# aidanmrli/rwm-pt-pytorch

Hardware: AMD Instinct MI355X
Metric: chain-MH-steps/sec (higher is better)
Workload: dtype f32; 1 GPU; BASELINE configs[2]: PT-RWM HIP, RoughCarpet dim=30 modes[-15,0,15], Normal proposal 2.38^2/dim, 32 geometric temps 1->0.01, swap_every=10, 65536 ladders per GPU; dim=30, temps=32, ladders_per_gpu=65536, mh_steps_per_launch=2000, swap_every=10, swap_mode=exchange, swap_order=sequential, rng=Philox4x32-10 in-kernel, world_size=1

## Files before the change

### include/ptrwm.h

```cpp
#ifndef PTRWM_H
#define PTRWM_H

#include <stdint.h>

#ifdef __cplusplus
extern "C" {
#endif

#define PTRWM_ABI_VERSION 3
#define PTRWM_SPLIT_NO_SWEEP 1
#define PTRWM_MAX_DIM 104
#define PTRWM_MAX_TEMPS 256

enum {
  PTRWM_OK = 0,
  PTRWM_E_NULL = -1,
  PTRWM_E_DIM = -2,
  PTRWM_E_TEMPS = -3,
  PTRWM_E_KIND = -4,
  PTRWM_E_ARG = -5,
  PTRWM_E_STRUCT = -6,
  PTRWM_E_LAUNCH = -7,
  PTRWM_E_NOVARIANT = -8
};
// ... 140 lines not shown
  uint32_t struct_size;
  int32_t temps;
  int32_t every;
  double *sum;
  double *sum_sq;
  double *sum_logp;
  int64_t *count;
} ptrwm_chain_moments_args;

int32_t ptrwm_run_with_chain_moments(const ptrwm_target_desc *target, const ptrwm_proposal_desc *proposal,
                                     const ptrwm_run_args *args, const ptrwm_chain_moments_args *chain_moments, void *stream);

int32_t ptrwm_split_chain_moments(const ptrwm_run_args *args, int32_t dim, const ptrwm_chain_moments_args *chain_moments,
                                  void *stream);

int32_t ptrwm_swap_sweep(const ptrwm_run_args *args, int32_t dim, int64_t event_index, int32_t rng_stream,
                         void *stream);

int32_t ptrwm_split_propose(const ptrwm_proposal_desc *proposal, const ptrwm_run_args *args, int32_t dim,
                            float *proposals, float *accept_u, void *stream);
int32_t ptrwm_split_accept(const ptrwm_run_args *args, int32_t dim, float *proposals, const float *accept_u,
                           const float *logp_proposed, void *stream);
int32_t ptrwm_split_advance(const ptrwm_run_args *args, void *stream);

int32_t ptrwm_logdensity(const ptrwm_target_desc *target, const float *x, float *out, int64_t n,
                         void *stream);

int32_t ptrwm_propose(const ptrwm_proposal_desc *proposal, int32_t dim, int32_t n_temps, int64_t n,
                      const float *ext_raw, uint64_t seed, float *out, void *stream);

int32_t ptrwm_philox_raw(uint64_t seed, uint32_t c0, uint32_t c1, uint32_t c2, uint32_t c3,
                         int64_t n, uint32_t *out, void *stream);

int32_t ptrwm_has_variant(int32_t target_kind, int32_t proposal_kind, int32_t dim);

int32_t ptrwm_abi_version(void);
const char *ptrwm_strerror(int32_t code);

#ifdef __cplusplus
}
#endif
#endif
```

### rwm-pt-pytorch_amd/csrc/capi.hip

```cpp
#include <algorithm>
#include <cmath>

#include "../../include/ptrwm.h"
#include "variants.h"

namespace ptrwm {

struct VariantPair {
  const TargetVariants *narrow, *wide;
  RunLaunchFn run(int proposal, int dpi) const {
    const RunLaunchFn f = narrow->run[proposal][dpi];
    return f != nullptr ? f : wide->run[proposal][dpi];
  }
  LogpLaunchFn logp(int dpi) const {
    const LogpLaunchFn f = narrow->logp[dpi];
    return f != nullptr ? f : wide->logp[dpi];
  }
};

#include "form_table.inc"

static void form_lerp(const float *a, const float *b, float t, float *out, int n) {
  for (int i = 0; i < n; ++i) out[i] = a[i] + (b[i] - a[i]) * t;
}
// ... 216 lines not shown
}

static int specialised_form(const ptrwm_target_desc *t, int perm[3]) {
  if (t->kind == PTRWM_TARGET_ROUGH_CARPET) return rough_carpet_fold(t->p, perm) ? 2 : (rough_carpet_two_term(t->p) ? 1 : 0);
  if (t->kind == PTRWM_TARGET_THREE_MIXTURE) return t->ip[0] == 1 ? 1 : 0;
  return 0;
}

static TParams make_tparams(const ptrwm_target_desc *t) {
  TParams tp;
  for (int i = 0; i < 12; ++i) tp.p[i] = t->p[i];
  for (int i = 0; i < 4; ++i) tp.ip[i] = t->ip[i];
  tp.vec0 = t->vec0;
  tp.vec1 = t->vec1;
  tp.mask[0] = tp.mask[1] = 0;
  if (t->kind == PTRWM_TARGET_ROUGH_CARPET) {
    tp.p[7] = -(float)t->dim * 0.91893853320467274178f;
  }
  if (t->kind == PTRWM_TARGET_HYBRID_ROSENBROCK) {
    const int blk = t->ip[0] - 1;
    for (int i = 1; i < t->dim; ++i)
      if ((i - 1) % blk == 0) tp.mask[i >> 6] |= (1ull << (i & 63));
  }
  return tp;
}

__global__ void split_advance_kernel(long long *device_step, long long n) { *device_step += n; }

__global__ void philox_raw_kernel(uint32_t *__restrict__ out, long long n, uint32_t c0, uint32_t c1, uint32_t c2,
                                  uint32_t c3, uint32_t k0, uint32_t k1) {
  const long long i = (long long)blockIdx.x * blockDim.x + threadIdx.x;
  if (i >= n) return;
  const u32x4 r = philox4x32_10(c0 + (uint32_t)i, c1, c2, c3, k0, k1);
  out[4 * i + 0] = r.x;
  out[4 * i + 1] = r.y;
  out[4 * i + 2] = r.z;
  out[4 * i + 3] = r.w;
}

struct SweepArgs {
  float *state, *logp;
  const float *beta, *ext_swap_u;
  long long *swap_accept, *last_swap_ordinal;
  const float *prev;
  double *sq_jump;
  long long chain_offset, event_index;
  unsigned long long step;
  int n_temps, dim, swap_mode, swap_order, rng_stream, chunk;
  unsigned k0, k1;
  const long long *device_step;
  long long burn_in, swap_every, event_offset;
};
constexpr int kSweepLdsBytes = 32768;

template <class state_t>
__global__ void __launch_bounds__(256) swap_sweep_kernel(SweepArgs a) {
  if (a.device_step != nullptr) {
    const long long s0 = *a.device_step + (long long)a.step, sc = s0 + 1;
    if (!(sc > a.burn_in && sc % a.swap_every == 0)) return;
    a.step = (unsigned long long)s0;
    a.event_index = sc / a.swap_every - a.burn_in / a.swap_every - 1 + a.event_offset;
  }
  extern __shared__ __attribute__((aligned(16))) unsigned char s_sweep[];
  __shared__ float s_l[256], s_u[256];
  __shared__ int s_src[256];
  const int T = a.n_temps, D = a.dim, tid = threadIdx.x, nthr = blockDim.x;
// ... 831 lines not shown
  const int dpi = width_index_for_dim(dim);
  if (dpi < 0) return PTRWM_E_DIM;
  PParams pp;
  pp.dim_scale = proposal->dim_scale;
  pp.inv_dim = proposal->inv_dim;
  const int n_raw = ptrwm_ext_raw_per_step(proposal->kind, dim);
  const unsigned k0 = (unsigned)(seed & 0xffffffffull), k1 = (unsigned)(seed >> 32);
  hipError_t err;
  switch (proposal->kind) {
    case PTRWM_PROPOSAL_NORMAL:
      err = launch_propose<NormalProposal>(dpi, out, n, dim, n_temps, proposal->temp_scale, pp, ext_raw, n_raw, k0, k1, (hipStream_t)stream);
      break;
    case PTRWM_PROPOSAL_LAPLACE:
      err = launch_propose<LaplaceProposal>(dpi, out, n, dim, n_temps, proposal->temp_scale, pp, ext_raw, n_raw, k0, k1, (hipStream_t)stream);
      break;
    default:
      err = launch_propose<UniformRadiusProposal>(dpi, out, n, dim, n_temps, proposal->temp_scale, pp, ext_raw, n_raw, k0, k1, (hipStream_t)stream);
      break;
  }
  return err == hipSuccess ? PTRWM_OK : PTRWM_E_LAUNCH;
}

int32_t ptrwm_philox_raw(uint64_t seed, uint32_t c0, uint32_t c1, uint32_t c2, uint32_t c3, int64_t n, uint32_t *out,
                         void *stream) {
  if (n < 0) return PTRWM_E_ARG;
  if (n == 0) return PTRWM_OK;
  if (out == nullptr) return PTRWM_E_NULL;
  const unsigned grid = (unsigned)((n + 255) / 256);
  hipLaunchKernelGGL(philox_raw_kernel, dim3(grid), dim3(256), 0, (hipStream_t)stream, out, (long long)n, c0, c1, c2,
                     c3, (unsigned)(seed & 0xffffffffull), (unsigned)(seed >> 32));
  return hipGetLastError() == hipSuccess ? PTRWM_OK : PTRWM_E_LAUNCH;
}

}
```

### rwm-pt-pytorch_amd/csrc/kernel.h

```cpp
#pragma once
#include "philox.h"
#include "proposals.h"
#include "targets.h"

namespace ptrwm {

#ifndef PTRWM_BLOCK_THREADS
#define PTRWM_BLOCK_THREADS 256
#endif
constexpr int kBlockThreads = PTRWM_BLOCK_THREADS;
constexpr int kWavesPerBlock = kBlockThreads / 64;
struct StepLdsWords {
  static constexpr int kSwapWords = 3;
  static constexpr int kParkedInts = 3;
  static constexpr int kExtraPerThread = kSwapWords + kParkedInts + 2;
  static constexpr int kStreamSlabs = 2;
  static constexpr int kStreamStatPerThread = 5;
  static constexpr unsigned kVoteBytes = 16u;
  static constexpr int floats_per_thread(int dp, bool stream) { return (stream ? kStreamSlabs * (dp + kStreamStatPerThread) : dp) + kExtraPerThread; }
  static constexpr unsigned bytes(int threads, int dp, bool stream, bool wide) { return (unsigned)(threads * floats_per_thread(dp, stream)) * 4u + (wide ? kVoteBytes : 0u); }
};
template <int DP, bool STREAM = false>
struct StepLds : StepLdsWords {
  static constexpr int kWaveFloats = 64 * floats_per_thread(DP, STREAM);
// ... 279 lines not shown
      else sum_logp[row0 + i] = reg[2 * rd + i];
    }
}

template <bool EXACT>
__device__ __forceinline__ int fresh_dim(int d0) {
  if constexpr (!EXACT) PTRWM_VALUE_BARRIER("+s"(d0));
  return d0;
}

typedef const __attribute__((address_space(4))) KArgs *kargs_ptr;
__device__ __forceinline__ kargs_ptr late_args() {
  uintptr_t p = (uintptr_t)__builtin_amdgcn_kernarg_segment_ptr();
  PTRWM_VALUE_BARRIER("+s"(p));
  return (kargs_ptr)p;
}

#ifndef PTRWM_J2_FENCE_MASK
#define PTRWM_J2_FENCE_MASK 7
#endif
#ifndef PTRWM_WAVES_SMALL
#define PTRWM_WAVES_SMALL 4
#endif
#ifndef PTRWM_WAVES_40
#define PTRWM_WAVES_40 3
#endif
#ifndef PTRWM_WAVES_MID
#define PTRWM_WAVES_MID 2
#endif
constexpr int min_waves_per_simd(int dp) {
  return dp <= 30 ? PTRWM_WAVES_SMALL : (dp <= 44 ? PTRWM_WAVES_40 : (dp <= 64 ? PTRWM_WAVES_MID : 1));
}
constexpr bool step_loop_at_register_cap(int dp, bool stream) { return !stream && min_waves_per_simd(dp) >= 4 && dp > 24; }

constexpr int stream_waves_per_simd(int dp) {
  return dp <= 10 ? 4 : (dp <= 20 ? 2 : (dp <= 30 ? 2 : 1));
}

constexpr int stream_register_waves(int dp) { return stream_waves_per_simd(dp) < 2 ? 2 : stream_waves_per_simd(dp); }

template <class Target, class Proposal, int DP, bool EXACT, bool FULL, bool STREAM = false>
__global__ void __launch_bounds__(kBlockThreads, STREAM ? stream_register_waves(DP) : min_waves_per_simd(DP)) ptrwm_step_kernel(const KArgs a) {
  static_assert(!(STREAM && FULL), "the streaming form is a production kernel: no fixture / trace arguments");
  const int T = a.n_temps;
  const int D0 = EXACT ? DP : a.dim;
  const int cpw = a.chains_per_wave;
  const bool wide = !STREAM && T > 64;
  const int wave = wave_in_block();
  const int tid = wide ? (int)threadIdx.x : (int)(threadIdx.x & 63);
  long long group = STREAM ? (long long)blockIdx.x * kWavesPerBlock + wave
                           : (wide ? (long long)blockIdx.x : (long long)blockIdx.x * kWavesPerBlock + (threadIdx.x >> 6));
  [[maybe_unused]] const long long n_groups = STREAM ? a.n_chains / cpw : 0;
  [[maybe_unused]] const long long group_stride = STREAM ? (long long)gridDim.x * kWavesPerBlock : 0;
  if (STREAM ? (group >= n_groups) : (group * cpw >= a.n_chains)) return;
  extern __shared__ __attribute__((aligned(16))) float s_dyn[];
  typedef float pf_vec4 __attribute__((ext_vector_type(4)));
  typedef StepLds<DP, STREAM> L;
  constexpr int NV = STREAM ? L::kSlabVectorsPerLane : 1;
  constexpr int kWaveFloats = L::kWaveFloats;
  [[maybe_unused]] int cur = 0;
  typedef const __attribute__((address_space(1))) void *dma_src;
  typedef __attribute__((address_space(3))) void *dma_dst;
  [[maybe_unused]] auto prefetch = [&](long long g, int slab) {
    const int tid = thread_index_now(wave) & 63;
    const kargs_ptr ap = late_args();
    const int n_vec = (cpw * T * D0) >> 2;
// ... 98 lines not shown
    }
    if constexpr (STREAM) asm volatile("s_waitcnt vmcnt(0)" ::: "memory");
    sync_group();
    const float *row = s_stage + row_head + (live ? tid : 0) * D0;
#pragma unroll
    for (int d = 0; d < DP; ++d) x[d] = (d < D0) ? row[d] : 0.0f;
  }
  float lp;
  [[maybe_unused]] double sq_old = 0.0;
  [[maybe_unused]] long long acc_old = 0;
  if constexpr (STREAM) {
    {
      const float *zone = s_dyn + wave * kWaveFloats + L::zone(cur);
      lp = (zone + L::kZoneLogp)[tid];
      if (a.sq_jump != nullptr) sq_old = reinterpret_cast<const double *>(zone + L::kZoneSqJump)[tid < cpw * T ? tid : 0];
      if (a.n_accept != nullptr) acc_old = reinterpret_cast<const long long *>(zone + L::kZoneAccept)[tid < cpw * T ? tid : 0];
    }
    if (have_pending) flush_pending();
    if (group + group_stride < n_groups) prefetch(group + group_stride, cur ^ 1);
  } else {
    lp = a.logp[rep];
  }
  const float beta_t = STREAM ? beta_t_s : a.beta[t];
  const float tscale = STREAM ? tscale_s : a.temp_scale[t];
  bool jump_trusted = false;
  if constexpr (Proposal::kKnowsJump) {
    float xmax = 0.0f;
#pragma unroll
    for (int d = 0; d < DP; ++d) xmax = __builtin_fmaxf(xmax, __builtin_fabsf(x[d]));
    jump_trusted = xmax <= kJumpTrust * Proposal::increment_scale(tscale, a.pp);
  }

  const unsigned long long gchain = (unsigned long long)(a.chain_offset + chain);
  RngCtx rc;
  rc.c2 = (uint32_t)gchain;
  rc.k0 = a.k0;
  rc.k1 = a.k1;
  const uint32_t c3_base = (uint32_t)t | ((uint32_t)(gchain >> 32) << 12);

  unsigned n_acc = 0;
  {
    const int gt = wide ? ((T + 63) & ~63) : 64;
    int *const park = reinterpret_cast<int *>(STREAM ? s_dyn + wave * kWaveFloats + L::parked(gt) : s_stage + L::parked(gt)) + tid;
    park[0] = (int)c3_base;
    park[L::kSwapCount * gt] = 0;
    park[L::kLastEvent * gt] = -1;
    reinterpret_cast<double *>(park - tid + L::kSqJump * gt)[tid] = 0.0;
  }

  const bool ext = FULL && a.full.ext_prop != nullptr;
  const bool trace_on =
      FULL && live && a.full.trace != nullptr && (chain < a.full.trace_chains) && (t < a.full.trace_temps);
  int to_swap = a.steps_to_swap;
  int to_trace = FULL ? a.full.steps_to_trace : 0;
  [[maybe_unused]] int to_mom = FULL ? a.full.steps_to_mom : 0;
  int trace_rows = 0;
  int swap_in_call = 0;
  const int ev_par0 = (int)(a.first_swap_event & 1);
  unsigned long long s = (unsigned long long)a.step0;

  constexpr int W = canon_width(DP);
  auto commit_plain = [&](bool acc, float jump, int jump_kind, int D) __attribute__((always_inline)) -> float {
    float j2;
    if (jump_kind != kJumpNone) {
      float from_states = 0.0f;
      if (!jump_trusted) {
        PTRWM_COLD_PATH();
        float j2p[4] = {0.0f, 0.0f, 0.0f, 0.0f};
        PTRWM_DIM_LOOP(d, DP, D, {
          const float dl = sub_rn(y[d], x[d]);
          j2p[d / W] = fmaf(dl, dl, j2p[d / W]);
        })
        from_states = tree4_add(j2p);
      }
      PTRWM_DIM_LOOP(d, DP, D, {
        x[d] = acc ? y[d] : x[d];
        if ((d & PTRWM_J2_FENCE_MASK) == PTRWM_J2_FENCE_MASK) sched_fence_soft();
      })
      j2 = acc ? (jump_trusted ? jump : from_states) : 0.0f;
    } else {
      float j2p[4] = {0.0f, 0.0f, 0.0f, 0.0f};
      PTRWM_DIM_LOOP(d, DP, D, {
        const float dl = sub_rn(y[d], x[d]);
        j2p[d / W] = fmaf(dl, dl, j2p[d / W]);
        x[d] = acc ? y[d] : x[d];
        if ((d & PTRWM_J2_FENCE_MASK) == PTRWM_J2_FENCE_MASK) sched_fence_soft();
      })
      j2 = tree4_add(j2p);
      if (!acc) j2 = 0.0f;
    }
    return j2;
  };
// ... 29 lines not shown
        if (mom_now && count_on && live && t < a.full.mom_temps) {
          const int mt = a.full.mom_temps, pc = a.full.mom_chain;
          const int m_rows = moments_rows(pc != 0, cpw, mt), m_row = pc != 0 ? cw * mt + t : t;
          double *const reg = L::moments_region(s_dyn, wide, wide ? ((T + 63) & ~63) : 64, wave, (int)moments_region_doubles(m_rows, D));
          double *const rs = reg + m_row * D;
          double *const rq = reg + (m_rows + m_row) * D;
          PTRWM_DIM_LOOP(d, DP, D, {
            const double v = (double)x[d];
            moments_add(rs + d, v);
            moments_add(rq + d, v * v);
          })
          moments_add(reg + 2 * m_rows * D + m_row, (double)lp);
        }
      }
    }
  };

  int i = 0;
  while (i < a.n_steps) {
    const int left = a.n_steps - i;
    const bool to_multiple = to_swap <= left;
    int run = to_multiple ? to_swap : left;
    to_swap = to_multiple ? a.swap_every : to_swap - left;
    bool count_on, acc;
    float lp_mh;
    float jump;
    int jump_kind;
    int D;
    for (;; ++i, ++s) {
      count_on = i >= a.burn_left;
      rc.c0hi = (uint32_t)(s >> 32) << 16;
      rc.c1 = (uint32_t)s;
      rc.c3 = c3_base | (kStreamMH << 8);
      if constexpr (step_loop_at_register_cap(DP, STREAM)) asm volatile("" : "+v"(rc.c2));

      long long srep = 0;
      const float *ext_raw = nullptr;
      float ext_u = 0.0f;
      if constexpr (FULL) {
        srep = ((long long)i * a.n_chains + chain) * T + t;
        if (ext) {
          ext_raw = a.full.ext_prop + srep * a.full.n_raw_ext;
          ext_u = a.full.ext_u[srep];
        }
      }

      jump = 0.0f;
      const float u_acc = Proposal::propose(y, x, fresh_dim<EXACT>(D0), tscale, a.pp, rc, ext_raw, ext_u, jump, jump_kind);
      const float lp_new = Target::template logp<false>(y, fresh_dim<EXACT>(D0), a.tp);
      D = fresh_dim<EXACT>(D0);

      acc = mh_accept(beta_t, lp_new, lp, u_acc);
      lp_mh = acc ? lp_new : lp;
      if constexpr (FULL) {
        if (a.full.accept_flags != nullptr && live) a.full.accept_flags[srep] = acc ? 1 : 0;
      }

      if (--run == 0) break;
      const float j2 = commit_plain(acc, jump, jump_kind, D);
      lp = lp_mh;
      finish_step(count_on, acc, j2, D);
    }
    const bool swap_due = to_multiple && count_on && (T > 1);

    float j2;
    if (!swap_due) {
      j2 = commit_plain(acc, jump, jump_kind, D);
// ... 273 lines not shown
```

### rwm-pt-pytorch_amd/csrc/philox.h

```cpp
#pragma once
#include <hip/hip_runtime.h>
#include <stdint.h>

namespace ptrwm {

struct u32x4 {
  uint32_t x, y, z, w;
};

constexpr uint32_t kPhiloxM0 = 0xD2511F53u;
constexpr uint32_t kPhiloxM1 = 0xCD9E8D57u;
constexpr uint32_t kPhiloxW0 = 0x9E3779B9u;
constexpr uint32_t kPhiloxW1 = 0xBB67AE85u;

constexpr uint32_t kStreamMH = 0u;
constexpr uint32_t kStreamSwap = 1u;

__device__ __forceinline__ void mul_hilo(uint32_t m, uint32_t x, uint32_t &hi, uint32_t &lo) {
  const uint64_t p = (uint64_t)m * x;
  hi = (uint32_t)(p >> 32);
  lo = (uint32_t)p;
}

__device__ __forceinline__ u32x4 philox4x32_10(uint32_t c0, uint32_t c1, uint32_t c2, uint32_t c3,
                                               uint32_t k0, uint32_t k1) {
#pragma unroll
  for (int r = 0; r < 10; ++r) {
    uint32_t hi0, lo0, hi1, lo1;
    mul_hilo(kPhiloxM0, c0, hi0, lo0);
    mul_hilo(kPhiloxM1, c2, hi1, lo1);
    uint32_t n0, n2;
    if (r >= 2) {
      n0 = __builtin_amdgcn_bitop3_b32(hi1, c1, k0, 0x96);
      n2 = __builtin_amdgcn_bitop3_b32(hi0, c3, k1, 0x96);
    } else {
      n0 = hi1 ^ c1 ^ k0;
      n2 = hi0 ^ c3 ^ k1;
    }
    c1 = lo1;
    c3 = lo0;
    c0 = n0;
    c2 = n2;
    k0 += kPhiloxW0;
    k1 += kPhiloxW1;
  }
  return u32x4{c0, c1, c2, c3};
}

#ifdef PTRWM_NO_VALUE_BARRIERS
#define PTRWM_VALUE_BARRIER(...) ((void)0)
#else
#define PTRWM_VALUE_BARRIER(...) asm volatile("" : __VA_ARGS__)
#endif

#define PTRWM_COLD_PATH() asm volatile("; ptrwm-cold-path")

typedef const __attribute__((address_space(4))) float *const_float_ptr;
__device__ __forceinline__ const_float_ptr uniform_vec(const float *p) {
  uintptr_t v = (uintptr_t)p;
  PTRWM_VALUE_BARRIER("+s"(v));
  return (const_float_ptr)v;
}

__device__ __forceinline__ const_float_ptr uniform_vec_again(const_float_ptr p) {
  uintptr_t v = (uintptr_t)p;
  PTRWM_VALUE_BARRIER("+s"(v));
  return (const_float_ptr)v;
}

__device__ __forceinline__ float u01(uint32_t r) { return (float)(r >> 8) * 0x1p-24f; }
__device__ __forceinline__ float u01_open0(uint32_t r) {
  return ((float)(r >> 8) + 1.0f) * 0x1p-24f;
}

constexpr float kLn2 = 0.69314718055994530942f;
// ... 60 lines not shown
```

### rwm-pt-pytorch_amd/csrc/proposals.h

```cpp
#pragma once
#include "philox.h"
#include "../../include/ptrwm.h"

namespace ptrwm {

struct RngCtx {
  uint32_t c0hi, c1, c2, c3, k0, k1;
};

enum { kJumpNone = 0, kJumpPartial = 1, kJumpTotal = 2 };
constexpr float kJumpTrust = 256.0f;

struct PParams {
  const float *__restrict__ dim_scale;
  float inv_dim;
};

__device__ __forceinline__ uint32_t pick(const u32x4 &r, int lane4) {
  return lane4 == 0 ? r.x : (lane4 == 1 ? r.y : (lane4 == 2 ? r.z : r.w));
}

template <int DP>
__device__ __forceinline__ void philox_normals(float (&z)[DP], int D, const RngCtx &rc, int w_a,
                                               float &ua, float &ub) {
  constexpr int NB = (2 * ((DP + 1) / 2)) / 4 + 1;
#pragma unroll
  for (int c = 0; c < NB; ++c) {
    if (4 * c + 4 <= DP && 4 * c + 4 <= D) {
      const u32x4 r = philox4x32_10(rc.c0hi | (uint32_t)c, rc.c1, rc.c2, rc.c3, rc.k0, rc.k1);
#pragma unroll
      for (int h = 0; h < 2; ++h) {
        const int d = (4 * c + 2 * h + 1 < DP) ? 4 * c + 2 * h : 0;
        float z0, z1;
        box_muller(h ? r.z : r.x, h ? r.w : r.y, z0, z1);
        z[d] = z0;
        z[d + 1] = z1;
      }
      sched_fence();
    } else if (4 * c <= w_a + 1) {
      const u32x4 r = philox4x32_10(rc.c0hi | (uint32_t)c, rc.c1, rc.c2, rc.c3, rc.k0, rc.k1);
      if (4 * c < DP && 4 * c < D) {
        float z0, z1;
        box_muller(r.x, r.y, z0, z1);
        z[4 * c < DP ? 4 * c : 0] = z0;
        if (4 * c + 1 < DP && 4 * c + 1 < D) z[4 * c + 1 < DP ? 4 * c + 1 : 0] = z1;
      }
      if (4 * c + 2 < DP && 4 * c + 2 < D) {
        float z0, z1;
        box_muller(r.z, r.w, z0, z1);
        z[4 * c + 2 < DP ? 4 * c + 2 : 0] = z0;
        if (4 * c + 3 < DP && 4 * c + 3 < D) z[4 * c + 3 < DP ? 4 * c + 3 : 0] = z1;
      }
      if (4 * c == w_a) {
        ua = u01(r.x);
        ub = u01(r.y);
      }
      if (4 * c + 2 == w_a) {
        ua = u01(r.z);
        ub = u01(r.w);
      }
      sched_fence();
    }
  }
}

template <int DP>
__device__ __forceinline__ float philox_normal_step(float (&y)[DP], const float (&x)[DP], int D, float tscale,
                                                    const RngCtx &rc, float &jump_total) {
  constexpr int W = canon_width(DP);
  float jump[4] = {0.0f, 0.0f, 0.0f, 0.0f};
  const float c_t = mul_rn(mul_rn(-2.0f * kLn2, tscale), tscale);
  constexpr int NB = (2 * ((DP + 1) / 2)) / 4 + 1;
#ifdef PTRWM_INJECT_ACCEPT_WORD_SLIP
  const int w_a = 2 * ((D + 1) >> 1) - 2;
#else
  const int w_a = 2 * ((D + 1) >> 1);
#endif
  float u_acc = 0.0f;
#pragma unroll
  for (int c = 0; c < NB; ++c) {
    if (4 * c + 4 <= DP && 4 * c + 4 <= D) {
      const u32x4 r = philox4x32_10(rc.c0hi | (uint32_t)c, rc.c1, rc.c2, rc.c3, rc.k0, rc.k1);
#pragma unroll
      for (int h = 0; h < 2; ++h) {
        const int d = (4 * c + 2 * h + 1 < DP) ? 4 * c + 2 * h : 0;
        const uint32_t ra = h ? r.z : r.x, rb = h ? r.w : r.y;
        const float arg = mul_rn(c_t, hw_log2(u01_open0(ra)));
        const float rad = hw_sqrt(arg);
        const float ang = bm_turns(rb);
        y[d] = fmaf(rad, __builtin_amdgcn_sinf(ang), x[d]);
        y[d + 1] = fmaf(rad, __builtin_amdgcn_cosf(ang), x[d + 1]);
        jump[d / W] = add_rn(jump[d / W], arg);
      }
      sched_fence();
    } else if (4 * c <= w_a) {
      const u32x4 r = philox4x32_10(rc.c0hi | (uint32_t)c, rc.c1, rc.c2, rc.c3, rc.k0, rc.k1);
#pragma unroll
      for (int h = 0; h < 2; ++h) {
        const int d = 4 * c + 2 * h;
        const uint32_t ra = h ? r.z : r.x, rb = h ? r.w : r.y;
        if (d < DP && d < D) {
          const float arg = mul_rn(c_t, hw_log2(u01_open0(ra)));
          const float rad = hw_sqrt(arg);
          const float ang = bm_turns(rb);
          const int d0 = d < DP ? d : 0, d1 = d + 1 < DP ? d + 1 : 0;
          const float sn = __builtin_amdgcn_sinf(ang);
          y[d0] = fmaf(rad, sn, x[d0]);
          if (d + 1 < DP && d + 1 < D) {
            y[d1] = fmaf(rad, __builtin_amdgcn_cosf(ang), x[d1]);
            jump[d0 / W] = add_rn(jump[d0 / W], arg);
          } else {
            const float i0 = mul_rn(rad, sn);
            jump[d0 / W] = fmaf(i0, i0, jump[d0 / W]);
          }
        }
        if (d == w_a) u_acc = u01(ra);
      }
      sched_fence();
    }
  }
  jump_total = tree4_add(jump);
  return u_acc;
}

template <int DP>
struct NormalProposal {
  static constexpr int kKind = PTRWM_PROPOSAL_NORMAL;
  static constexpr bool kKnowsJump = true;
  __device__ __forceinline__ static float increment_scale(float tscale, const PParams &) { return tscale; }
  __device__ __forceinline__ static float propose(float (&y)[DP], const float (&x)[DP], int D,
                                                  float tscale, const PParams &, const RngCtx &rc,
                                                  const float *ext_raw, float ext_u, float &jump, int &jump_kind) {
    float u_acc = ext_u;
    if (ext_raw != nullptr) {
      jump_kind = kJumpNone;
#pragma unroll
      for (int d = 0; d < DP; ++d)
        if (d < D) y[d] = add_rn(x[d], mul_rn(ext_raw[d], tscale));
    } else {
      jump_kind = kJumpTotal;
      u_acc = philox_normal_step<DP>(y, x, D, tscale, rc, jump);
    }
    return u_acc;
  }
};

template <int DP>
struct LaplaceProposal {
  static constexpr int kKind = PTRWM_PROPOSAL_LAPLACE;
  static constexpr bool kKnowsJump = false;
  __device__ __forceinline__ static float increment_scale(float tscale, const PParams &) { return tscale; }
  __device__ __forceinline__ static float transform(float u01v, float scale) {
    const float u = u01v - 0.5f;
    const float au = __builtin_fabsf(u);
    const float arg = __builtin_fmaxf(-2.0f * au, -0.999999f);
    const float l1p = hw_log2(1.0f + arg) * kLn2;
    const float t = mul_rn(scale, l1p);
    return __builtin_bit_cast(float, __builtin_amdgcn_bitop3_b32(__builtin_bit_cast(uint32_t, t),
                                                                 __builtin_bit_cast(uint32_t, u), 0x80000000u, 0xd2));
  }
  __device__ __forceinline__ static float propose(float (&y)[DP], const float (&x)[DP], int D,
                                                  float tscale, const PParams &pp, const RngCtx &rc,
                                                  const float *ext_raw, float ext_u, float &, int &jump_kind) {
    float u_acc = ext_u;
    jump_kind = kJumpNone;
    const const_float_ptr dsc = uniform_vec(pp.dim_scale);
    if (ext_raw != nullptr) {
#pragma unroll
      for (int d = 0; d < DP; ++d)
        if (d < D) y[d] = add_rn(x[d], transform(ext_raw[d], mul_rn(dsc[d], tscale)));
    } else {
      constexpr int NB = DP / 4 + 1;
#pragma unroll
      for (int c = 0; c < NB; ++c) {
        if (4 * c + 4 <= DP && 4 * c + 4 <= D) {
          const u32x4 r = philox4x32_10(rc.c0hi | (uint32_t)c, rc.c1, rc.c2, rc.c3, rc.k0, rc.k1);
#pragma unroll
          for (int q = 0; q < 4; ++q) {
            const int d = (4 * c + q < DP) ? 4 * c + q : 0;
            y[d] = add_rn(x[d], transform(u01(pick(r, q)), mul_rn(dsc[d], tscale)));
          }
          sched_fence();
        } else if (4 * c <= D) {
          const u32x4 r = philox4x32_10(rc.c0hi | (uint32_t)c, rc.c1, rc.c2, rc.c3, rc.k0, rc.k1);
#pragma unroll
          for (int q = 0; q < 4; ++q) {
            const int d = 4 * c + q;
            if (d < DP && d < D) {
              const int ds = d < DP ? d : 0;
              y[ds] = add_rn(x[ds], transform(u01(pick(r, q)), mul_rn(dsc[ds], tscale)));
            }
            if (d == D) u_acc = u01(pick(r, q));
          }
          sched_fence();
        }
      }
    }
    return u_acc;
  }
};

template <int DP>
struct UniformRadiusProposal {
  static constexpr int kKind = PTRWM_PROPOSAL_UNIFORM_RADIUS;
  static constexpr bool kKnowsJump = true;
  __device__ __forceinline__ static float increment_scale(float tscale, const PParams &pp) { return tscale * hw_sqrt(pp.inv_dim); }
  __device__ __forceinline__ static float propose(float (&y)[DP], const float (&x)[DP], int D,
                                                  float tscale, const PParams &pp, const RngCtx &rc,
                                                  const float *ext_raw, float ext_u, float &jump, int &jump_kind) {
    float u_acc = ext_u, u_rad;
    if (ext_raw != nullptr) {
#pragma unroll
      for (int d = 0; d < DP; ++d)
        if (d < D) y[d] = ext_raw[d];
      u_rad = ext_raw[D];
    } else {
      float ua = 0.0f, ub = 0.0f;
      philox_normals<DP>(y, D, rc, 2 * ((D + 1) >> 1), ua, ub);
      u_rad = ua;
      u_acc = ub;
    }
    constexpr int W = canon_width(DP);
    float n2p[4] = {0.0f, 0.0f, 0.0f, 0.0f};
    PTRWM_DIM_LOOP(d, DP, D, { n2p[d / W] = fmaf(y[d], y[d], n2p[d / W]); })
    const float nrm_sq = tree4_add(n2p);
    const float nrm = hw_sqrt(nrm_sq);
    const float safe = nrm > 1e-12f ? nrm : 1.0f;
    const float rad = tscale * hw_exp2(pp.inv_dim * hw_log2(u_rad));
    const float inv = div_rn(1.0f, safe);
    if (ext_raw != nullptr) {
      jump_kind = kJumpNone;
#pragma unroll
      for (int d = 0; d < DP; ++d)
        if (d < D) y[d] = add_rn(x[d], mul_rn(mul_rn(y[d], inv), rad));
    } else {
      const float k = mul_rn(inv, rad);
#pragma unroll
      for (int d = 0; d < DP; ++d)
        if (d < D) y[d] = fmaf(y[d], k, x[d]);
      jump_kind = kJumpTotal;
      jump = mul_rn(mul_rn(nrm_sq, k), k);
    }
    return u_acc;
  }
};

}
```

### rwm-pt-pytorch_amd/ptrwm_hip/__init__.py

```python
from __future__ import annotations

import ctypes as C
import os
from dataclasses import dataclass
from typing import Optional

import torch

_HERE = os.path.dirname(os.path.abspath(__file__))
LIB_PATH = os.environ.get("PTRWM_LIB") or os.path.join(os.path.dirname(_HERE), "lib", "libptrwm_hip.so")

ABI_VERSION = 3
MAX_DIM = 104
MAX_TEMPS = 256

TARGET_ROUGH_CARPET = 0
TARGET_THREE_MIXTURE = 1
TARGET_FULL_ROSENBROCK = 2
TARGET_EVEN_ROSENBROCK = 3
TARGET_HYBRID_ROSENBROCK = 4
TARGET_IID_GAMMA = 5
TARGET_IID_BETA = 6
TARGET_DIAG_GAUSSIAN = 7
TARGET_HYPERCUBE = 8
# ... 113 lines not shown
    "ptrwm_last_launch_kind": (C.c_int32, []),
    "ptrwm_last_launch_functor": (C.c_int32, []),
    "ptrwm_has_quad_variant": (C.c_int32, [C.c_int32, C.c_int32, C.c_int32, C.c_int32]),
    "ptrwm_has_thread_variant": (C.c_int32, [C.c_int32, C.c_int32, C.c_int32]),
    "ptrwm_auto_form": (C.c_int32, [C.c_int32, C.c_int32, C.c_int32, C.c_int32, C.c_int64]),
    "ptrwm_auto_form_for": (C.c_int32, [C.c_int32, C.c_int32, C.c_int32, C.c_int32, C.c_int64, C.c_int32]),
    "ptrwm_device_simds": (C.c_int32, [C.c_void_p]),
    "ptrwm_source_hash": (C.c_char_p, []),
    "ptrwm_form_table_source_hash": (C.c_char_p, []),
    "ptrwm_run": (C.c_int32, [C.POINTER(TargetDesc), C.POINTER(ProposalDesc), C.POINTER(RunArgs), C.c_void_p]),
    "ptrwm_run_with_moments": (
        C.c_int32,
        [C.POINTER(TargetDesc), C.POINTER(ProposalDesc), C.POINTER(RunArgs), C.POINTER(MomentsArgs), C.c_void_p]),
    "ptrwm_split_moments": (C.c_int32, [C.POINTER(RunArgs), C.c_int32, C.POINTER(MomentsArgs), C.c_void_p]),
    "ptrwm_run_with_chain_moments": (
        C.c_int32,
        [C.POINTER(TargetDesc), C.POINTER(ProposalDesc), C.POINTER(RunArgs), C.POINTER(ChainMomentsArgs), C.c_void_p]),
    "ptrwm_split_chain_moments": (C.c_int32, [C.POINTER(RunArgs), C.c_int32, C.POINTER(ChainMomentsArgs), C.c_void_p]),
    "ptrwm_swap_sweep": (C.c_int32, [C.POINTER(RunArgs), C.c_int32, C.c_int64, C.c_int32, C.c_void_p]),
    "ptrwm_split_propose": (
        C.c_int32, [C.POINTER(ProposalDesc), C.POINTER(RunArgs), C.c_int32, C.c_void_p, C.c_void_p, C.c_void_p]),
    "ptrwm_split_accept": (
        C.c_int32, [C.POINTER(RunArgs), C.c_int32, C.c_void_p, C.c_void_p, C.c_void_p, C.c_void_p]),
    "ptrwm_split_advance": (C.c_int32, [C.POINTER(RunArgs), C.c_void_p]),
    "ptrwm_logdensity": (C.c_int32, [C.POINTER(TargetDesc), C.c_void_p, C.c_void_p, C.c_int64, C.c_void_p]),
    "ptrwm_propose": (
        C.c_int32,
        [C.POINTER(ProposalDesc), C.c_int32, C.c_int32, C.c_int64, C.c_void_p, C.c_uint64, C.c_void_p, C.c_void_p],
    ),
    "ptrwm_philox_raw": (
        C.c_int32,
        [C.c_uint64, C.c_uint32, C.c_uint32, C.c_uint32, C.c_uint32, C.c_int64, C.c_void_p, C.c_void_p],
    ),
}

_lib = None


def load_library(path: Optional[str] = None):
    global _lib
    if _lib is not None and path is None:
        return _lib
    p = path or LIB_PATH
    if not os.path.exists(p):
        raise RuntimeError(
            f"HIP engine library not found at {p}. Build it first: "
            "`python -c 'import __graft_entry__ as g; g.build()'` or `make -C rwm-pt-pytorch_amd/csrc`. "
            "There is no CPU fallback."
        )
    lib = C.CDLL(p)
    lib.ptrwm_abi_version.restype, lib.ptrwm_abi_version.argtypes = SYMBOLS["ptrwm_abi_version"]
    if lib.ptrwm_abi_version() != ABI_VERSION:
        raise RuntimeError(f"ABI mismatch: library {p} is version {lib.ptrwm_abi_version()}, this binding {ABI_VERSION} "
                           "(rebuild: make -C rwm-pt-pytorch_amd/csrc)")
    for name, (restype, argtypes) in SYMBOLS.items():
        fn = getattr(lib, name)
        fn.restype = restype
        fn.argtypes = argtypes
    form = os.environ.get("PTRWM_KERNEL_FORM")
    if form:
        lib.ptrwm_set_kernel_form({"auto": FORM_AUTO, "thread": FORM_THREAD, "quad": FORM_QUAD}[form.lower()])
    smode = os.environ.get("PTRWM_STREAM")
    if smode:
        lib.ptrwm_set_stream_mode({"auto": STREAM_AUTO, "off": STREAM_OFF, "on": STREAM_ON}[smode.lower()])
    if path is None:
        _lib = lib
# ... 205 lines not shown
    with on_device(x.device):
        rc = lib.ptrwm_logdensity(C.byref(desc), xp, out.data_ptr(), x.shape[0], _stream(x.device))
    if rc != 0:
        raise PTRWMError(rc, "ptrwm_logdensity")
    return out


def propose(proposal: Proposal, dim: int, n: int, seed: int = 0, ext_raw: Optional[torch.Tensor] = None) -> torch.Tensor:
    lib = load_library()
    T = proposal.temp_scale.numel()
    dev = proposal.temp_scale.device
    desc = proposal.desc()
    if ext_raw is not None:
        if tuple(ext_raw.shape) != (n, T, ext_raw_per_step(proposal.kind, dim)):
            raise ValueError(f"ext_raw has shape {tuple(ext_raw.shape)}")
    out = torch.empty(n, T, dim, device=dev, dtype=torch.float32)
    with on_device(dev):
        rc = lib.ptrwm_propose(C.byref(desc), dim, T, n, _opt(ext_raw, "ext_raw", torch.float32), seed & (2**64 - 1),
                               out.data_ptr(), _stream(dev))
    if rc != 0:
        raise PTRWMError(rc, "ptrwm_propose")
    return out


def philox_raw(seed: int, c0: int, c1: int, c2: int, c3: int, n: int, device) -> torch.Tensor:
    lib = load_library()
    out = torch.empty(n, 4, device=device, dtype=torch.int32)
    if not out.is_cuda:
        raise RuntimeError("philox_raw needs a ROCm device")
    with on_device(out.device):
        rc = lib.ptrwm_philox_raw(seed, c0, c1, c2, c3, n, out.data_ptr(), _stream(out.device))
    if rc != 0:
        raise PTRWMError(rc, "ptrwm_philox_raw")
    return out.to(torch.int64) & 0xFFFFFFFF


class RunPlan:

    def __init__(
        self,
        target: Target,
        proposal: Proposal,
        *,
        state: torch.Tensor,
        logp: torch.Tensor,
        beta: torch.Tensor,
        burn_in: int = 0,
        swap_every: int = 1,
        swap_mode: int = SWAP_EXCHANGE,
        swap_order: int = ORDER_SEQUENTIAL,
        seed: int = 0,
        chain_offset: int = 0,
        n_accept: Optional[torch.Tensor] = None,
        sq_jump: Optional[torch.Tensor] = None,
        swap_accept: Optional[torch.Tensor] = None,
        last_swap_ordinal: Optional[torch.Tensor] = None,
    ):
        self._lib = load_library()
        if isinstance(state, torch.Tensor) and state.dtype not in (torch.float32, torch.float64):
            raise TypeError(f"state must be torch.float32 or torch.float64, got {state.dtype}")
        self.state_dtype = state.dtype if isinstance(state, torch.Tensor) else torch.float32
        if state.dim() != 3:
            raise ValueError("state must be [n_chains, n_temps, dim]")
        Cn, T, D = state.shape
        if target is not None and D != target.dim:
            raise ValueError(f"state dim {D} != target dim {target.dim}")
# ... 317 lines not shown
```

Before: 47.31 billion chain-MH-steps/s.

## Precompute step-invariant Philox rounds per chain and reuse across MH steps

Splits Philox4x32-10 so the parts of the first rounds that depend only on the chain, the stream constant and the high step bits are computed once per block index and kept in registers. Each MH step then finishes the remaining rounds from this cached head plus a per-step shared term. The goal is to cut integer multiply work in the in-kernel RNG, which dominates cheap targets like RoughCarpet. The cost is extra VGPRs per cached block, capped by a register-budget heuristic that allows 5 blocks at the register cap. A raw test entry point is added to check the result against the original Philox.

```diff
diff --git a/include/ptrwm.h b/include/ptrwm.h
--- a/include/ptrwm.h
+++ b/include/ptrwm.h
@@ -196,6 +196,9 @@
 int32_t ptrwm_philox_raw(uint64_t seed, uint32_t c0, uint32_t c1, uint32_t c2, uint32_t c3,
                          int64_t n, uint32_t *out, void *stream);
 
+int32_t ptrwm_philox_raw_head(uint64_t seed, uint64_t step, uint32_t c2, uint32_t c3, int64_t n,
+                              uint32_t *out, void *stream);
+
 int32_t ptrwm_has_variant(int32_t target_kind, int32_t proposal_kind, int32_t dim);
 
 int32_t ptrwm_abi_version(void);
diff --git a/rwm-pt-pytorch_amd/csrc/capi.hip b/rwm-pt-pytorch_amd/csrc/capi.hip
--- a/rwm-pt-pytorch_amd/csrc/capi.hip
+++ b/rwm-pt-pytorch_amd/csrc/capi.hip
@@ -272,6 +272,20 @@
   const long long i = (long long)blockIdx.x * blockDim.x + threadIdx.x;
   if (i >= n) return;
   const u32x4 r = philox4x32_10(c0 + (uint32_t)i, c1, c2, c3, k0, k1);
+  out[4 * i + 0] = r.x;
+  out[4 * i + 1] = r.y;
+  out[4 * i + 2] = r.z;
+  out[4 * i + 3] = r.w;
+}
+
+__global__ void philox_raw_head_kernel(uint32_t *__restrict__ out, long long n, unsigned long long step, uint32_t c2, uint32_t c3,
+                                       uint32_t k0, uint32_t k1) {
+  const long long i = (long long)blockIdx.x * blockDim.x + threadIdx.x;
+  if (i >= n) return;
+  const uint32_t step_hi = (uint32_t)(step >> 32);
+  const PhiloxHead hd = philox_head(step_hi, c2, c3, k0, k1, (uint32_t)i);
+  const PhiloxStep st = philox_step_shared((uint32_t)step, c2, k0);
+  const u32x4 r = philox4x32_10_from_head(hd, st, (uint32_t)i | (step_hi << 16), k0, k1);
   out[4 * i + 0] = r.x;
   out[4 * i + 1] = r.y;
   out[4 * i + 2] = r.z;
@@ -1169,4 +1183,14 @@
   return hipGetLastError() == hipSuccess ? PTRWM_OK : PTRWM_E_LAUNCH;
 }
 
-}
+int32_t ptrwm_philox_raw_head(uint64_t seed, uint64_t step, uint32_t c2, uint32_t c3, int64_t n, uint32_t *out, void *stream) {
+  if (n < 0 || n > 65536) return PTRWM_E_ARG;
+  if (n == 0) return PTRWM_OK;
+  if (out == nullptr) return PTRWM_E_NULL;
+  const unsigned grid = (unsigned)((n + 255) / 256);
+  hipLaunchKernelGGL(philox_raw_head_kernel, dim3(grid), dim3(256), 0, (hipStream_t)stream, out, (long long)n,
+                     (unsigned long long)step, c2, c3, (unsigned)(seed & 0xffffffffull), (unsigned)(seed >> 32));
+  return hipGetLastError() == hipSuccess ? PTRWM_OK : PTRWM_E_LAUNCH;
+}
+
+}
diff --git a/rwm-pt-pytorch_amd/csrc/kernel.h b/rwm-pt-pytorch_amd/csrc/kernel.h
--- a/rwm-pt-pytorch_amd/csrc/kernel.h
+++ b/rwm-pt-pytorch_amd/csrc/kernel.h
@@ -335,6 +335,16 @@
   return dp <= 30 ? PTRWM_WAVES_SMALL : (dp <= 44 ? PTRWM_WAVES_40 : (dp <= 64 ? PTRWM_WAVES_MID : 1));
 }
 constexpr bool step_loop_at_register_cap(int dp, bool stream) { return !stream && min_waves_per_simd(dp) >= 4 && dp > 24; }
+
+#ifndef PTRWM_HEAD_BLOCKS_AT_CAP
+#define PTRWM_HEAD_BLOCKS_AT_CAP 5
+#endif
+constexpr int philox_head_blocks(int dp, int waves_per_simd, int blocks) {
+  const int vgprs = waves_per_simd >= 4 ? 128 : (waves_per_simd == 3 ? 168 : 256);
+  const int spare = vgprs - (2 * dp + 50);
+  const int fit = step_loop_at_register_cap(dp, false) ? PTRWM_HEAD_BLOCKS_AT_CAP : (spare < 0 ? 0 : spare / 3);
+  return fit < blocks ? fit : blocks;
+}
 
 constexpr int stream_waves_per_simd(int dp) {
   return dp <= 10 ? 4 : (dp <= 20 ? 2 : (dp <= 30 ? 2 : 1));
@@ -499,7 +509,8 @@
   }
 
   const unsigned long long gchain = (unsigned long long)(a.chain_offset + chain);
-  RngCtx rc;
+  constexpr int NH = (STREAM || !EXACT) ? 0 : philox_head_blocks(DP, min_waves_per_simd(DP), Proposal::kBlocks);
+  typename RngCtxFor<NH>::type rc;
   rc.c2 = (uint32_t)gchain;
   rc.k0 = a.k0;
   rc.k1 = a.k1;
@@ -525,6 +536,11 @@
   int swap_in_call = 0;
   const int ev_par0 = (int)(a.first_swap_event & 1);
   unsigned long long s = (unsigned long long)a.step0;
+  if constexpr (NH > 0) {
+#pragma unroll
+    for (int b = 0; b < NH; ++b) rc.head[b] = PhiloxHead{0u, 0u, 0u};
+  }
+  [[maybe_unused]] uint32_t head_hi = (uint32_t)(s >> 32) + 1u;
 
   constexpr int W = canon_width(DP);
   auto commit_plain = [&](bool acc, float jump, int jump_kind, int D) __attribute__((always_inline)) -> float {
@@ -620,7 +636,18 @@
       rc.c0hi = (uint32_t)(s >> 32) << 16;
       rc.c1 = (uint32_t)s;
       rc.c3 = c3_base | (kStreamMH << 8);
-      if constexpr (step_loop_at_register_cap(DP, STREAM)) asm volatile("" : "+v"(rc.c2));
+      if constexpr (NH > 0) {
+        const uint32_t s_hi = (uint32_t)(s >> 32);
+        if (s_hi != head_hi) {
+          PTRWM_COLD_PATH();
+          head_hi = s_hi;
+#pragma unroll
+          for (int b = 0; b < NH; ++b) rc.head[b] = philox_head(s_hi, rc.c2, rc.c3, rc.k0, rc.k1, (uint32_t)b);
+        }
+        rc.step = philox_step_shared(rc.c1, rc.c2, rc.k0);
+      } else if constexpr (step_loop_at_register_cap(DP, STREAM)) {
+        asm volatile("" : "+v"(rc.c2));
+      }
 
       long long srep = 0;
       const float *ext_raw = nullptr;
diff --git a/rwm-pt-pytorch_amd/csrc/philox.h b/rwm-pt-pytorch_amd/csrc/philox.h
--- a/rwm-pt-pytorch_amd/csrc/philox.h
+++ b/rwm-pt-pytorch_amd/csrc/philox.h
@@ -41,6 +41,63 @@
     c3 = lo0;
     c0 = n0;
     c2 = n2;
+    k0 += kPhiloxW0;
+    k1 += kPhiloxW1;
+  }
+  return u32x4{c0, c1, c2, c3};
+}
+
+struct PhiloxHead {
+  uint32_t a;
+  uint32_t b;
+  uint32_t c;
+};
+struct PhiloxStep {
+  uint32_t hi, lo;
+};
+
+__device__ __forceinline__ PhiloxHead philox_head(uint32_t step_hi, uint32_t c2, uint32_t c3, uint32_t k0, uint32_t k1,
+                                                  uint32_t block) {
+  uint32_t hi0, lo0, hi1, lo1, h, l;
+  mul_hilo(kPhiloxM0, block | (step_hi << 16), hi0, lo0);
+  mul_hilo(kPhiloxM1, c2, hi1, lo1);
+  mul_hilo(kPhiloxM1, hi0 ^ c3 ^ k1, h, l);
+  const uint32_t c0pp = h ^ lo1 ^ (k0 + kPhiloxW0);
+  PhiloxHead hd;
+  hd.a = l ^ (k0 + 2u * kPhiloxW0);
+  mul_hilo(kPhiloxM0, c0pp, h, l);
+  hd.b = h ^ (k1 + 2u * kPhiloxW1);
+  hd.c = l;
+  return hd;
+}
+
+__device__ __forceinline__ PhiloxStep philox_step_shared(uint32_t c1, uint32_t c2, uint32_t k0) {
+  uint32_t hi1, lo1;
+  mul_hilo(kPhiloxM1, c2, hi1, lo1);
+  PhiloxStep st;
+  mul_hilo(kPhiloxM0, hi1 ^ c1 ^ k0, st.hi, st.lo);
+  return st;
+}
+
+__device__ __forceinline__ u32x4 philox4x32_10_from_head(const PhiloxHead &hd, const PhiloxStep &st, uint32_t c0,
+                                                         uint32_t k0, uint32_t k1) {
+  uint32_t c2 = st.hi ^ ((kPhiloxM0 * c0) ^ (k1 + kPhiloxW1));
+  uint32_t hi1, c1, c3;
+  mul_hilo(kPhiloxM1, c2, hi1, c1);
+  c0 = hi1 ^ hd.a;
+  c2 = hd.b ^ st.lo;
+  c3 = hd.c;
+  k0 += 3u * kPhiloxW0;
+  k1 += 3u * kPhiloxW1;
+#pragma unroll
+  for (int r = 3; r < 10; ++r) {
+    uint32_t hi0, lo0, lo1;
+    mul_hilo(kPhiloxM0, c0, hi0, lo0);
+    mul_hilo(kPhiloxM1, c2, hi1, lo1);
+    c0 = __builtin_amdgcn_bitop3_b32(hi1, c1, k0, 0x96);
+    c2 = __builtin_amdgcn_bitop3_b32(hi0, c3, k1, 0x96);
+    c1 = lo1;
+    c3 = lo0;
     k0 += kPhiloxW0;
     k1 += kPhiloxW1;
   }
diff --git a/rwm-pt-pytorch_amd/csrc/proposals.h b/rwm-pt-pytorch_amd/csrc/proposals.h
--- a/rwm-pt-pytorch_amd/csrc/proposals.h
+++ b/rwm-pt-pytorch_amd/csrc/proposals.h
@@ -5,8 +5,34 @@
 namespace ptrwm {
 
 struct RngCtx {
+  static constexpr int kHeads = 0;
   uint32_t c0hi, c1, c2, c3, k0, k1;
 };
+template <int NH>
+struct RngCtxHeads : RngCtx {
+  static_assert(NH > 0, "no heads: RngCtx");
+  static constexpr int kHeads = NH;
+  PhiloxStep step;
+  PhiloxHead head[NH];
+};
+
+template <int NH>
+struct RngCtxFor {
+  using type = RngCtxHeads<NH>;
+};
+template <>
+struct RngCtxFor<0> {
+  using type = RngCtx;
+};
+
+template <class Rc>
+__device__ __forceinline__ u32x4 step_block(const Rc &rc, int c) {
+  const uint32_t c0 = rc.c0hi | (uint32_t)c;
+  if constexpr (Rc::kHeads > 0) {
+    if (c < Rc::kHeads) return philox4x32_10_from_head(rc.head[c], rc.step, c0, rc.k0, rc.k1);
+  }
+  return philox4x32_10(c0, rc.c1, rc.c2, rc.c3, rc.k0, rc.k1);
+}
 
 enum { kJumpNone = 0, kJumpPartial = 1, kJumpTotal = 2 };
 constexpr float kJumpTrust = 256.0f;
@@ -20,14 +46,14 @@
   return lane4 == 0 ? r.x : (lane4 == 1 ? r.y : (lane4 == 2 ? r.z : r.w));
 }
 
-template <int DP>
-__device__ __forceinline__ void philox_normals(float (&z)[DP], int D, const RngCtx &rc, int w_a,
+template <int DP, class Rc>
+__device__ __forceinline__ void philox_normals(float (&z)[DP], int D, const Rc &rc, int w_a,
                                                float &ua, float &ub) {
   constexpr int NB = (2 * ((DP + 1) / 2)) / 4 + 1;
 #pragma unroll
   for (int c = 0; c < NB; ++c) {
     if (4 * c + 4 <= DP && 4 * c + 4 <= D) {
-      const u32x4 r = philox4x32_10(rc.c0hi | (uint32_t)c, rc.c1, rc.c2, rc.c3, rc.k0, rc.k1);
+      const u32x4 r = step_block(rc, c);
 #pragma unroll
       for (int h = 0; h < 2; ++h) {
         const int d = (4 * c + 2 * h + 1 < DP) ? 4 * c + 2 * h : 0;
@@ -38,7 +64,7 @@
       }
       sched_fence();
     } else if (4 * c <= w_a + 1) {
-      const u32x4 r = philox4x32_10(rc.c0hi | (uint32_t)c, rc.c1, rc.c2, rc.c3, rc.k0, rc.k1);
+      const u32x4 r = step_block(rc, c);
       if (4 * c < DP && 4 * c < D) {
         float z0, z1;
         box_muller(r.x, r.y, z0, z1);
@@ -64,9 +90,9 @@
   }
 }
 
-template <int DP>
+template <int DP, class Rc>
 __device__ __forceinline__ float philox_normal_step(float (&y)[DP], const float (&x)[DP], int D, float tscale,
-                                                    const RngCtx &rc, float &jump_total) {
+                                                    const Rc &rc, float &jump_total) {
   constexpr int W = canon_width(DP);
   float jump[4] = {0.0f, 0.0f, 0.0f, 0.0f};
   const float c_t = mul_rn(mul_rn(-2.0f * kLn2, tscale), tscale);
@@ -80,7 +106,7 @@
 #pragma unroll
   for (int c = 0; c < NB; ++c) {
     if (4 * c + 4 <= DP && 4 * c + 4 <= D) {
-      const u32x4 r = philox4x32_10(rc.c0hi | (uint32_t)c, rc.c1, rc.c2, rc.c3, rc.k0, rc.k1);
+      const u32x4 r = step_block(rc, c);
 #pragma unroll
       for (int h = 0; h < 2; ++h) {
         const int d = (4 * c + 2 * h + 1 < DP) ? 4 * c + 2 * h : 0;
@@ -94,7 +120,7 @@
       }
       sched_fence();
     } else if (4 * c <= w_a) {
-      const u32x4 r = philox4x32_10(rc.c0hi | (uint32_t)c, rc.c1, rc.c2, rc.c3, rc.k0, rc.k1);
+      const u32x4 r = step_block(rc, c);
 #pragma unroll
       for (int h = 0; h < 2; ++h) {
         const int d = 4 * c + 2 * h;
@@ -126,10 +152,12 @@
 template <int DP>
 struct NormalProposal {
   static constexpr int kKind = PTRWM_PROPOSAL_NORMAL;
+  static constexpr int kBlocks = (2 * ((DP + 1) / 2)) / 4 + 1;
   static constexpr bool kKnowsJump = true;
   __device__ __forceinline__ static float increment_scale(float tscale, const PParams &) { return tscale; }
+  template <class Rc>
   __device__ __forceinline__ static float propose(float (&y)[DP], const float (&x)[DP], int D,
-                                                  float tscale, const PParams &, const RngCtx &rc,
+                                                  float tscale, const PParams &, const Rc &rc,
                                                   const float *ext_raw, float ext_u, float &jump, int &jump_kind) {
     float u_acc = ext_u;
     if (ext_raw != nullptr) {
@@ -139,7 +167,7 @@
         if (d < D) y[d] = add_rn(x[d], mul_rn(ext_raw[d], tscale));
     } else {
       jump_kind = kJumpTotal;
-      u_acc = philox_normal_step<DP>(y, x, D, tscale, rc, jump);
+      u_acc = philox_normal_step(y, x, D, tscale, rc, jump);
     }
     return u_acc;
   }
@@ -148,6 +176,7 @@
 template <int DP>
 struct LaplaceProposal {
   static constexpr int kKind = PTRWM_PROPOSAL_LAPLACE;
+  static constexpr int kBlocks = DP / 4 + 1;
   static constexpr bool kKnowsJump = false;
   __device__ __forceinline__ static float increment_scale(float tscale, const PParams &) { return tscale; }
   __device__ __forceinline__ static float transform(float u01v, float scale) {
@@ -159,8 +188,9 @@
     return __builtin_bit_cast(float, __builtin_amdgcn_bitop3_b32(__builtin_bit_cast(uint32_t, t),
                                                                  __builtin_bit_cast(uint32_t, u), 0x80000000u, 0xd2));
   }
+  template <class Rc>
   __device__ __forceinline__ static float propose(float (&y)[DP], const float (&x)[DP], int D,
-                                                  float tscale, const PParams &pp, const RngCtx &rc,
+                                                  float tscale, const PParams &pp, const Rc &rc,
                                                   const float *ext_raw, float ext_u, float &, int &jump_kind) {
     float u_acc = ext_u;
     jump_kind = kJumpNone;
@@ -174,7 +204,7 @@
 #pragma unroll
       for (int c = 0; c < NB; ++c) {
         if (4 * c + 4 <= DP && 4 * c + 4 <= D) {
-          const u32x4 r = philox4x32_10(rc.c0hi | (uint32_t)c, rc.c1, rc.c2, rc.c3, rc.k0, rc.k1);
+          const u32x4 r = step_block(rc, c);
 #pragma unroll
           for (int q = 0; q < 4; ++q) {
             const int d = (4 * c + q < DP) ? 4 * c + q : 0;
@@ -182,7 +212,7 @@
           }
           sched_fence();
         } else if (4 * c <= D) {
-          const u32x4 r = philox4x32_10(rc.c0hi | (uint32_t)c, rc.c1, rc.c2, rc.c3, rc.k0, rc.k1);
+          const u32x4 r = step_block(rc, c);
 #pragma unroll
           for (int q = 0; q < 4; ++q) {
             const int d = 4 * c + q;
@@ -203,10 +233,12 @@
 template <int DP>
 struct UniformRadiusProposal {
   static constexpr int kKind = PTRWM_PROPOSAL_UNIFORM_RADIUS;
+  static constexpr int kBlocks = (2 * ((DP + 1) / 2)) / 4 + 1;
   static constexpr bool kKnowsJump = true;
   __device__ __forceinline__ static float increment_scale(float tscale, const PParams &pp) { return tscale * hw_sqrt(pp.inv_dim); }
+  template <class Rc>
   __device__ __forceinline__ static float propose(float (&y)[DP], const float (&x)[DP], int D,
-                                                  float tscale, const PParams &pp, const RngCtx &rc,
+                                                  float tscale, const PParams &pp, const Rc &rc,
                                                   const float *ext_raw, float ext_u, float &jump, int &jump_kind) {
     float u_acc = ext_u, u_rad;
     if (ext_raw != nullptr) {
@@ -216,7 +248,7 @@
       u_rad = ext_raw[D];
     } else {
       float ua = 0.0f, ub = 0.0f;
-      philox_normals<DP>(y, D, rc, 2 * ((D + 1) >> 1), ua, ub);
+      philox_normals(y, D, rc, 2 * ((D + 1) >> 1), ua, ub);
       u_rad = ua;
       u_acc = ub;
     }
diff --git a/rwm-pt-pytorch_amd/ptrwm_hip/__init__.py b/rwm-pt-pytorch_amd/ptrwm_hip/__init__.py
--- a/rwm-pt-pytorch_amd/ptrwm_hip/__init__.py
+++ b/rwm-pt-pytorch_amd/ptrwm_hip/__init__.py
@@ -169,6 +169,8 @@
         C.c_int32,
         [C.c_uint64, C.c_uint32, C.c_uint32, C.c_uint32, C.c_uint32, C.c_int64, C.c_void_p, C.c_void_p],
     ),
+    "ptrwm_philox_raw_head": (
+        C.c_int32, [C.c_uint64, C.c_uint64, C.c_uint32, C.c_uint32, C.c_int64, C.c_void_p, C.c_void_p]),
 }
 
 _lib = None
@@ -440,6 +442,18 @@
         rc = lib.ptrwm_philox_raw(seed, c0, c1, c2, c3, n, out.data_ptr(), _stream(out.device))
     if rc != 0:
         raise PTRWMError(rc, "ptrwm_philox_raw")
+    return out.to(torch.int64) & 0xFFFFFFFF
+
+
+def philox_raw_head(seed: int, step: int, c2: int, c3: int, n: int, device) -> torch.Tensor:
+    lib = load_library()
+    out = torch.empty(n, 4, device=device, dtype=torch.int32)
+    if not out.is_cuda:
+        raise RuntimeError("philox_raw_head needs a ROCm device")
+    with on_device(out.device):
+        rc = lib.ptrwm_philox_raw_head(seed, step, c2, c3, n, out.data_ptr(), _stream(out.device))
+    if rc != 0:
+        raise PTRWMError(rc, "ptrwm_philox_raw_head")
     return out.to(torch.int64) & 0xFFFFFFFF
 
 
```

New measurement: 46.10 billion chain-MH-steps/s. -2.6%, worse.
